# yangzhaojason/DualDiff

Hardware: AMD Instinct MI355X
Metric: denoising-steps/sec, 6-view 224×400 fp16, 50-step DDIM @ 1/2/4/8 MI355X (higher is better)
Workload: dtype fp16; 1 GPU; BASELINE configs[1]: 6-view 224x400 (28x50 latents) multiview UNet + 2 ControlNet branches (ORS panorama + ORS-3D, SFA on), CFG 2.0 -> 12 view-instances/scene, DDIM-50 schedule, random-init weights; scenes_per_gpu=1, parallelism=scene-sharded x1 (no data-path collective), hip_graph=True, streams=3, invariant_conditioning=recomputed every step

## Files before the change

### dualdiff_amd/_native.py

```python
import ctypes
import os

import torch
from ctypes import (POINTER, Structure, c_char_p, c_float, c_int32, c_int64, c_uint32, c_void_p)

from . import _build

DD_F16, DD_BF16, DD_F32 = 0, 1, 2
DD_EPI_NONE, DD_EPI_GEGLU, DD_EPI_SILU = 0, 1, 2


class GemmDesc(Structure):
    _fields_ = [
        ("a", c_void_p), ("a2", c_void_p), ("lda", c_int64), ("lda2", c_int64), ("k1", c_int32),
        ("rows", c_int32), ("n", c_int32), ("k", c_int32),
        ("w", c_void_p), ("bias", c_void_p), ("rowvec", c_void_p),
        ("rows_per_inst", c_int32), ("ld_rowvec", c_int32),
        ("res", c_void_p), ("ldres", c_int64),
        ("out", c_void_p), ("ldc", c_int64),
        ("alpha", c_float), ("accumulate", c_int32), ("epilogue", c_int32),
        ("conv", c_int32), ("hin", c_int32), ("win", c_int32), ("cin", c_int32),
        ("hv", c_int32), ("wv", c_int32), ("hout", c_int32), ("wout", c_int32), ("stride", c_int32),
        ("dtype", c_int32), ("tile", c_int32), ("split_k", c_int32),
        ("ws", c_void_p), ("ws_bytes", c_int64),
# ... 69 lines not shown
    "dd_gemm_num_tiles": (c_int32, []),
    "dd_gemm_tile_id": (c_int32, [c_int32]),
    "dd_gemm_kernel_name": (c_char_p, [POINTER(GemmDesc)]),
    "dd_gemm_conv_pad": (c_int32, [POINTER(GemmDesc), c_int32, c_void_p]),
    "dd_gemm_conv_pad_workspace_bytes": (c_int64, [POINTER(GemmDesc), c_int32]),
    "dd_gemm_conv_pad_kernel_name": (c_char_p, [POINTER(GemmDesc), c_int32]),
    "dd_groupnorm_nhwc": (c_int32, [c_void_p, c_int32, c_void_p, c_int32, c_void_p, c_void_p, c_void_p,
                                    c_int32, c_int32, c_int32, c_float, c_int32, c_int32,
                                    c_void_p, c_int64, c_void_p]),
    "dd_groupnorm_workspace_bytes": (c_int64, [c_int32, c_int32]),
    "dd_groupnorm_is_fused": (c_int32, [c_int32, c_int32, c_int32]),
    "dd_layernorm": (c_int32, [c_void_p, c_void_p, c_void_p, c_void_p, c_int64, c_int32, c_float,
                               c_int32, c_void_p]),
    "dd_attention": (c_int32, [POINTER(AttnDesc), c_void_p]),
    "dd_attention_kernel_name": (c_char_p, [POINTER(AttnDesc)]),
    "dd_add": (c_int32, [c_void_p, c_void_p, c_void_p, c_void_p, c_int64, c_int32, c_void_p]),
    "dd_scale": (c_int32, [c_void_p, c_void_p, c_float, c_int64, c_int32, c_void_p]),
    "dd_probe_spin": (c_int32, [c_void_p, c_uint32, c_void_p]),
    "dd_groupnorm_splitk": (c_int32, [c_void_p, c_int32, c_void_p, c_void_p, c_int32, c_void_p, c_int64, c_void_p,
                                      c_void_p, c_void_p, c_void_p, c_int32, c_int32, c_int32, c_int32, c_float, c_int32,
                                      c_int32, c_void_p]),
    "dd_xattn320": (c_int32, [POINTER(XAttnDesc), c_void_p]),
    "dd_nchw_to_nhwc_views": (c_int32, [c_void_p, c_void_p, c_int32, c_int32, c_int32, c_int32, c_int32, c_int32, c_int32,
                                        c_void_p]),
    "dd_fourier_embed_strided": (c_int32, [c_void_p, c_void_p, c_int64, c_int32, POINTER(c_float), c_int32, c_int32,
                                           c_int32, c_int32, c_int32, c_int64, c_int64, c_int64, c_int64, c_void_p]),
    "dd_box_tokens": (c_int32, [POINTER(BoxTokensDesc), c_void_p]),
    "dd_ctx_assemble": (c_int32, [c_void_p, c_void_p, c_void_p, c_void_p, c_void_p, c_int32, c_int32, c_int32, c_int32,
                                  c_int32, c_int32, c_int32, c_int32, c_void_p]),
    "dd_gemm8": (c_int32, [POINTER(Gemm8Desc), c_void_p]),
    "dd_rowquant_fp8": (c_int32, [c_void_p, c_void_p, c_void_p, c_void_p, c_void_p, c_int64, c_int32, c_int64, c_float,
                                  c_int32, c_void_p]),
    "dd_xattn_pack_weight": (c_int32, [c_void_p, c_void_p, c_int32, c_void_p]),
    "dd_silu": (c_int32, [c_void_p, c_void_p, c_int64, c_int32, c_void_p]),
    "dd_nchw_to_nhwc": (c_int32, [c_void_p, c_void_p, c_int32, c_int32, c_int32, c_int32, c_int32, c_void_p]),
    "dd_nhwc_to_nchw": (c_int32, [c_void_p, c_void_p, c_int32, c_int32, c_int32, c_int32, c_int32, c_void_p]),
    "dd_timestep_embedding": (c_int32, [c_void_p, c_void_p, c_int32, c_int32, c_int32, c_float,
                                        c_int32, c_void_p]),
    "dd_cfg_unipc_step": (c_int32, [c_void_p, c_void_p, c_void_p, c_void_p, c_void_p, c_void_p, c_void_p, c_void_p,
                                    c_float, c_int64, c_int32, c_void_p]),
    "dd_softmax_rows": (c_int32, [c_void_p, c_void_p, c_int64, c_int32, c_int64, c_int64, c_int32, c_void_p]),
    "dd_ors_project": (c_int32, [c_void_p, c_void_p, c_void_p, c_void_p, c_void_p, c_int32, c_int32, c_int32,
                                 c_float, c_int32, c_int32, c_int32, c_void_p]),
    "dd_fourier_embed": (c_int32, [c_void_p, c_void_p, c_int64, c_int32, POINTER(c_float), c_int32, c_int32,
                                   c_int32, c_int32, c_void_p]),
    "dd_conv3x3_small_cout": (c_int32, [c_void_p, c_void_p, c_void_p, c_void_p, c_int32, c_int32,
                                        c_int32, c_int32, c_int32, c_int32, c_void_p]),
    "dd_vae_posterior": (c_int32, [c_void_p, c_void_p, c_void_p, c_void_p, c_void_p, c_int32, c_int32, c_int32, c_float,
                                   c_int32, c_int32, c_void_p]),
    "dd_image_quantize_u8": (c_int32, [c_void_p, c_void_p, c_int32, c_int32, c_int32, c_int32, c_int32, c_void_p]),
    "dd_image_resample_u8": (c_int32, [c_void_p, c_void_p, c_int32, c_int32, c_int32, c_int32, c_int32, c_void_p, c_void_p,
                                       c_int32, c_void_p, c_void_p, c_int32, c_int32, c_int32, c_int32, c_int32, c_int32,
                                       c_int32, c_int32, c_void_p]),
    "dd_image_load_u8": (c_int32, [c_void_p, c_void_p, c_int32, c_int32, c_int32, c_int32, c_int32, c_void_p, c_void_p,
                                   c_int32, c_void_p, c_void_p, c_int32, c_void_p, c_int32, c_int32, c_void_p]),
    "dd_clip_embed": (c_int32, [c_void_p, c_void_p, c_void_p, c_void_p, c_void_p, c_int32, c_int32, c_int32, c_int32,
                                c_int32, c_int32, c_void_p]),
    "dd_causal_attention": (c_int32, [c_void_p, c_void_p, c_void_p, c_void_p, c_int64, c_int64, c_int64, c_int64,
                                      c_int64, c_int64, c_int64, c_int64, c_int32, c_int32, c_int32, c_int32, c_float,
                                      c_int32, c_void_p]),
    "dd_conv3x3_thin": (c_int32, [c_void_p, c_void_p, c_void_p, c_void_p, c_int32, c_int32, c_int32, c_int32, c_int32,
                                  c_int32, c_int32, c_int32, c_void_p]),
    "dd_cfg_ddim_step": (c_int32, [c_void_p, c_void_p, c_void_p, c_void_p, c_void_p, c_float,
                                   c_int64, c_int32, c_void_p]),
    "dd_cfg_ddim_step_given": (c_int32, [c_void_p, c_void_p, c_void_p, c_void_p, c_void_p, c_float, c_void_p, c_void_p,
                                         c_void_p, c_void_p, c_int32, c_int64, c_int64, c_int32, c_void_p]),
# ... 55 lines not shown
```

### dualdiff_amd/csrc/xattn.hip

```cpp
#include "dd_common.h"
#include <type_traits>

namespace {

constexpr int XC = 320;
constexpr int XH = 8;
constexpr int XD = 40;
constexpr int XR = 80;
constexpr int XW = 10;
constexpr int XPITCH = XC + 8;
constexpr int XLK = 128;
constexpr size_t kActBytes = 53 * 1024;

struct XAttnParams {
  const void* x; int64_t ldx;
  const void* res; int64_t ldres;
  const void* wq; const void* wo;
  const void* bo;
  const void* k; const void* v;
  int64_t ldk, ldv;
  int64_t k_is, k_hs, v_is, v_hs;
  void* out; int64_t ldo;
  void* ln_out; int64_t ld_ln; const void* ln_g; const void* ln_b; float ln_eps;
  int inst, n, lk;
// ... 343 lines not shown
#pragma unroll
  for (int tm = 0; tm < 5; ++tm) {
    float a = 0.f;
#pragma unroll
    for (int w = 0; w < XW; ++w) a += red2[(tm * 16 + c) * XW + w];
    const float rstd = 1.0f / sqrtf(a * (1.0f / XC) + p.ln_eps);
    const int row = tm * 16 + c;
    if (row >= nrows) continue;
#pragma unroll
    for (int tn = 0; tn < 2; ++tn) {
      const int ch = wave * 32 + tn * 16 + g * 4;
      V4 o4;
#pragma unroll
      for (int r = 0; r < 4; ++r)
        o4[r] = (T)(((float)yv[tn][tm][r] - mean[tm]) * rstd * (float)lng[tn][r] + (float)lnb4[tn][r]);
      *reinterpret_cast<V4*>(lnb + (int64_t)row * p.ld_ln + ch) = o4;
    }
  }
}

constexpr size_t kXSmem = kActBytes + (size_t)4 * XC * 32 * 2;

template <typename T>
int launch_xattn(const XAttnParams& p, hipStream_t s) {
  static_assert(2 * (2 * XLK * XD * 2) == 4 * XC * 32, "two K/V buffers = the four weight slots");
  static_assert(XR * 41 * 16 <= 52 * 1024 && 53 * 1024 == (int)kActBytes && XPITCH * 2 == 41 * 16, "activation tile");
  auto kern = dd_xattn320_kernel<T>;
  static std::atomic<uint64_t> attr_done{0};
  dd_ensure_dyn_lds(reinterpret_cast<const void*>(kern), kXSmem, attr_done);
  hipLaunchKernelGGL(kern, dim3(p.inst * p.tiles), dim3(64 * XW), kXSmem, s, p);
  return dd_check_launch();
}

}

namespace {
template <typename T>
__global__ void dd_xattn_pack_kernel(const T* __restrict__ w, T* __restrict__ out) {
  const int q = blockIdx.x * blockDim.x + threadIdx.x;
  if (q >= 10 * XC * 4) return;
  const int ks = q / (XC * 4), rem = q - ks * (XC * 4);
  const int n = rem >> 2, pos = rem & 3;
  const int src = ks * 32 + ((pos ^ ((n >> 2) & 3)) << 3);
  dd_st16(out + (int64_t)q * 8, dd_ld16(w + (int64_t)n * XC + src));
}
}

extern "C" int dd_xattn_pack_weight(const void* w, void* packed, int32_t dtype, dd_stream_t stream) {
  if (!w || !packed || !dd_aligned16(w) || !dd_aligned16(packed)) return DD_ERR_BAD_ARG;
  if (dtype != DD_F16 && dtype != DD_BF16) return DD_ERR_BAD_ARG;
  dd_clear_error();
  const int chunks = 10 * XC * 4;
  return dd_dispatch16(dtype, [&](auto t) {
    using T = typename decltype(t)::type;
    hipLaunchKernelGGL(dd_xattn_pack_kernel<T>, dim3((chunks + 255) / 256), dim3(256), 0, dd_stream(stream),
                       (const T*)w, (T*)packed);
    return dd_check_launch();
  });
}

extern "C" int dd_xattn320(const dd_xattn_desc* d, dd_stream_t stream) {
  if (!d || !d->x || !d->wq || !d->wo || !d->bo || !d->k || !d->v || !d->out) return DD_ERR_BAD_ARG;
  if (d->instances <= 0 || d->rows_per_inst <= 0 || d->lk <= 0) return DD_ERR_BAD_ARG;
  if (d->channels != XC || d->heads != XH) return DD_ERR_UNSUPPORTED;
  if (d->lk > XLK) return DD_ERR_UNSUPPORTED;
  if (d->dtype != DD_F16 && d->dtype != DD_BF16) return DD_ERR_BAD_ARG;
// ... 26 lines not shown
```

### dualdiff_amd/networks/layers.py

```python
import math

import torch
import torch.nn as nn

from .. import ops as O


CACHE_EPOCH = [0]


class _Cached(nn.Module):

    def _drop_cache(self):
        CACHE_EPOCH[0] += 1
        for k in [k for k in self.__dict__ if k.startswith("_pk_")]:
            del self.__dict__[k]

    def _apply(self, fn, *a, **k):
        self._drop_cache()
        return super()._apply(fn, *a, **k)

    def _load_from_state_dict(self, *a, **k):
        self._drop_cache()
        return super()._load_from_state_dict(*a, **k)
# ... 66 lines not shown
    if not p.is_contiguous():
        if not x.is_cuda or x.dtype not in (torch.float16, torch.bfloat16):
            p = p.contiguous()
        else:
            return O.nchw_to_nhwc(x), m, h, w
    return p.reshape(m * h * w, c), m, h, w


def as_nchw_view(x2d, m, h, w):
    return x2d.view(m, h, w, x2d.shape[1]).permute(0, 3, 1, 2)


class Linear(_Cached):

    def __init__(self, in_features, out_features, bias=True, conv=False):
        super().__init__()
        self.in_features, self.out_features, self.conv = in_features, out_features, conv
        shape = (out_features, in_features, 1, 1) if conv else (out_features, in_features)
        self.weight = nn.Parameter(torch.empty(shape))
        self.bias = nn.Parameter(torch.empty(out_features)) if bias else None

    @property
    def w2d(self):
        if "_pk_w" not in self.__dict__:
            self.__dict__["_pk_w"] = _pad_cols(self.weight.detach().reshape(self.out_features, -1))
        return self.__dict__["_pk_w"]

    @property
    def wx(self):
        ver = (self.weight.data_ptr(), self.weight._version)
        hit = self.__dict__.get("_pk_wx")
        if hit is None or (hit[1] != ver and not torch.cuda.is_current_stream_capturing()):
            hit = self.__dict__["_pk_wx"] = (O.xattn_pack_weight(self.w2d), ver)
        return hit[0]

    fp8_mfma = False

    @property
    def w8p(self):
        if "_pk_w8p" not in self.__dict__:
            self.__dict__["_pk_w8p"] = O.quantize_fp8_padded(self.w2d)
        return self.__dict__["_pk_w8p"]

    def run(self, x2d, ln_next=None, **kw):
        if ln_next is not None and ln_producer_ok(self, ln_next, kw):
            w = self.w2d
            out = O.gemm(x2d, w, self.bias, ln_out=(ln_next.weight, ln_next.bias, ln_next.eps), **kw)
            out._ln_cache = (ln_next, out._ln_out)
            return out
        w = self.w2d
        if w.shape[1] != self.in_features:
            x2d = torch.nn.functional.pad(x2d, (0, w.shape[1] - x2d.shape[1]))
        return O.gemm(x2d, w, self.bias, **kw)

    def run_ln(self, x2d, norm, **kw):
        if self.fp8_mfma and fp8_mfma_ok(norm, self.in_features, self.out_features, x2d) \
                and set(kw) <= {"epilogue"} and kw.get("epilogue", O.DD_EPI_NONE) in (O.DD_EPI_NONE, O.DD_EPI_GEGLU):
            a8, sa = O.rowquant_fp8(x2d, (norm.weight, norm.bias, norm.eps))
            w8, sw = self.w8p
            return O.gemm8(a8, sa, w8, sw, self.bias, dtype=x2d.dtype, geglu=kw.get("epilogue") == O.DD_EPI_GEGLU)
        if not ln_fold_ok(norm, self.in_features, self.out_features, x2d):
            return self.run(norm.run(x2d), **kw)
        w, ln = fold_layernorm(self.__dict__, "_pk_ln", norm, [self.weight], [self.bias])
        return O.gemm(x2d, w, None, ln=ln, **kw)

    def forward(self, x):
# ... 86 lines not shown
def ln_fold_ok(norm, k, n=None, x=None):
    if LN_FOLD == "0" or not isinstance(norm, LayerNorm) or k not in (320, 640, 1280):
        return False
    if LN_FOLD == "stats":
        return x is not None and getattr(x, "_ln_stats", None) is not None
    return LN_FOLD == "all" or (n is not None and n <= k)


def want_ln_stats():
    return LN_FOLD == "stats"


LN_PRODUCER = __import__("os").environ.get("DD_LN_PRODUCER", "1") != "0"


def ln_producer_ok(lin, norm, kw):
    if not LN_PRODUCER or not isinstance(norm, LayerNorm) or lin.out_features != 320:
        return False
    if LN_FOLD != "0":
        return False
    if lin.w2d.shape[1] % 64 or kw.get("a2") is not None and kw["a2"].shape[1] % 64:
        return False
    bad = ("ln", "ln_stats", "head_major", "out_f32", "accumulate", "rowvec", "out", "tile", "split_k")
    return not any(kw.get(k) for k in bad) and kw.get("epilogue", O.DD_EPI_NONE) == O.DD_EPI_NONE \
        and kw.get("alpha", 1.0) == 1.0


def fp8_mfma_ok(norm, k, n, x2d):
    return isinstance(norm, LayerNorm) and k in (640, 1280) and n >= 3 * k and x2d.is_contiguous() \
        and getattr(x2d, "_ln_cache", None) is None


XATTN_FUSED = __import__("os").environ.get("DD_XATTN_FUSED", "1") != "0"


HEAD_MAJOR = __import__("os").environ.get("DD_ATTN_HEAD_MAJOR", "1") != "0"


def fold_layernorm(cache, key, norm, weights, biases):
    params = [norm.weight, norm.bias] + list(weights) + [b for b in biases if b is not None]
    ver = tuple((t._version, t.data_ptr()) for t in params)
    hit = cache.get(key)
    if hit is not None and hit[0] == ver:
        return hit[1], hit[2]
    with torch.no_grad():
        w = torch.cat([t.detach().reshape(t.shape[0], -1) for t in weights], dim=0).float()
        b = torch.cat([(bb.detach().float() if bb is not None else torch.zeros(t.shape[0], device=t.device))
                       for t, bb in zip(weights, biases)])
        wp = (w * norm.weight.detach().float()[None, :]).to(weights[0].dtype).contiguous()
        colsum = wp.float().sum(dim=1).contiguous()
        lnb = (w @ norm.bias.detach().float() + b).contiguous()
    cache[key] = (ver, wp, (colsum, lnb, norm.eps))
    return wp, (colsum, lnb, norm.eps)


class _Dropout(nn.Module):

    def forward(self, x):
        return x


class Timesteps(nn.Module):
    def __init__(self, num_channels, flip_sin_to_cos, downscale_freq_shift):
        super().__init__()
        self.num_channels, self.flip_sin_to_cos = num_channels, flip_sin_to_cos
        self.downscale_freq_shift = downscale_freq_shift
# ... 160 lines not shown
    def run_self(self, x2d, batch, lq, res=None, norm=None, ln_stats=False, ln_next=None):
        c, hd = self.inner_dim, self.heads
        if HEAD_MAJOR and self.to_q.bias is None:
            qkv = self.project_qkv(x2d, norm, head_major=True)
            o = O.attention(qkv[:hd], qkv[hd:2 * hd], qkv[2 * hd:], batch, lq, lq, hd, self.dim_head,
                            q_prescaled=True)
        else:
            qkv = self.project_qkv(x2d, norm)
            o = O.attention(qkv[:, :c], qkv[:, c:2 * c], qkv[:, 2 * c:], batch, lq, lq, hd,
                            self.dim_head, self.scale)
        return self.to_out[0].run(o, res=res, ln_stats=ln_stats, ln_next=ln_next)

    def run_cross(self, x2d, batch, lq, ctx2d, lk, res=None, kv=None, norm=None, ln_stats=False, ln_next=None):
        c = self.inner_dim
        pre = self.__dict__.pop("_kv_prefetched", None)
        if kv is None and pre is not None and pre[0] is ctx2d:
            kv, side = pre[1], pre[2]
            if side is not None:
                torch.cuda.current_stream().wait_stream(side)
                if not torch.cuda.is_current_stream_capturing():
                    kv.record_stream(torch.cuda.current_stream())
        if kv is None:
            kv = self.project_kv(ctx2d)
        lk_dev = lk_dev_for(ctx2d, lk)
        if XATTN_FUSED and O.xattn320_ok(c, self.heads, lk, x2d.shape[0]) and self.to_q.in_features == c and self.to_q.bias is None \
                and not ln_stats and LN_FOLD == "0":
            xn = x2d if norm is None else norm.run(x2d)
            lno = (ln_next.weight, ln_next.bias, ln_next.eps) if LN_PRODUCER and isinstance(ln_next, LayerNorm) else None
            out = O.xattn320(xn, self.to_q.wx, self.to_out[0].wx, self.to_out[0].bias, kv[:, :c], kv[:, c:], batch, lq,
                             lk, self.scale, res=res, ln_out=lno, lk_dev=lk_dev)
            if lno is not None:
                out._ln_cache = (ln_next, out._ln_out)
            return out
        q_hm = HEAD_MAJOR and self.to_q.bias is None
        kw = {"head_major": self._hm(self.heads)} if q_hm else {}
        q = self.to_q.run(x2d, **kw) if norm is None else self.to_q.run_ln(x2d, norm, **kw)
        o = O.attention(q, kv[:, :c], kv[:, c:], batch, lq, lk, self.heads, self.dim_head, self.scale,
                        q_prescaled=q_hm, lk_dev=lk_dev)
        return self.to_out[0].run(o, res=res, ln_stats=ln_stats, ln_next=ln_next)

    def forward(self, hidden_states, encoder_hidden_states=None, attention_mask=None, **kw):
        return self.processor(self, hidden_states, encoder_hidden_states=encoder_hidden_states,
                              attention_mask=attention_mask, **kw)


def enable_fp8_weights(model, on=True, mfma=True):
    if not mfma:
        raise NotImplementedError("the weights-only fp8 form (row-panel GEMM family) was removed in round 5; use mfma=True")
    n = 0
    for mod in model.modules():
        if isinstance(mod, Attention):
            mod.fp8_mfma = bool(on)
            mod._drop_cache()
            n += 1
        elif isinstance(mod, GEGLU):
            mod.proj.fp8_mfma = bool(on)
            mod.proj._drop_cache()
    return n


def prefetch_cross_kv(model, ctx2d, side):
    main = torch.cuda.current_stream()
    side.wait_stream(main)
    with torch.cuda.stream(side):
        for blk in model.modules():
            mod = getattr(blk, "attn2", None) if isinstance(blk, BasicTransformerBlock) else None
# ... 309 lines not shown
```

### dualdiff_amd/ops.py

```python
import collections as _collections
import ctypes
import os as _os

import torch

from . import _native, _timer, _workspace, tuning
from ._native import DD_BF16, DD_EPI_GEGLU, DD_EPI_NONE, DD_EPI_SILU, DD_F16, AttnDesc, Gemm8Desc, GemmDesc, XAttnDesc
from ._timer import KernelTimer, _stream, set_timer
from ._workspace import workspace, workspace_owner
from .tuning import (CHALLENGE_TILES, TUNE_TABLE_PATH, forget_tuned, load_tuned, save_tuned,
                     tune_candidates, tuned_table)

_THIN_CONV = _os.environ.get("DD_THIN_CONV", "1") != "0"
GN_SPLITK = _os.environ.get("DD_GN_SPLITK", "0") == "1"
LN_OUT_TILE = int(_os.environ.get("DD_LN_OUT_TILE", "0"))
XATTN_MAX_WGS = int(_os.environ.get("DD_XATTN_MAX_WGS", "256"))
CAUSAL_ATTN_MAX_L = 128
_ZERO_BIAS = {}
_FDT = {torch.float16: 0, torch.bfloat16: 1, torch.float32: 2}


def _dtype_code(dtype):
    if dtype == torch.float16:
        return DD_F16
    if dtype == torch.bfloat16:
        return DD_BF16
    raise TypeError("dualdiff_amd ops take fp16 / bf16 tensors, got %s" % dtype)


def _dt(t):
    return _dtype_code(t.dtype)


def _tname(code):
    return "f16" if code == DD_F16 else "bf16"


def _need_gpu(*ts):
    for t in ts:
        if t is not None and not t.is_cuda:
            raise RuntimeError("dualdiff_amd ops run on the GPU only (got a %s tensor); "
                               "there is no CPU fallback" % t.device)


def _ptr(t):
    return ctypes.c_void_p(t.data_ptr()) if t is not None else None


def _forget_derived(t):
# ... 541 lines not shown
    d.x, d.ldx = x.data_ptr(), x.stride(0)
    if res is not None:
        res = _rows2d(res)
        d.res, d.ldres = res.data_ptr(), res.stride(0)
    d.wq, d.wo = wqp.data_ptr(), wop.data_ptr()
    if bo is None:
        key = (x.dtype, x.device)
        if key not in _ZERO_BIAS:
            _ZERO_BIAS[key] = torch.zeros(320, dtype=x.dtype, device=x.device)
        bo = _ZERO_BIAS[key]
    d.bo = bo.data_ptr()
    d.k, d.ldk, d.k_inst_stride, d.k_head_stride = kv_operand(k)
    d.v, d.ldv, d.v_inst_stride, d.v_head_stride = kv_operand(v)
    d.out, d.ldo = out.data_ptr(), out.stride(0)
    d.instances, d.rows_per_inst, d.lk = int(instances), int(rows_per_inst), int(lk)
    d.channels, d.heads, d.scale, d.dtype = 320, 8, float(scale), _dt(x)
    d.lk_dev = lk_dev.data_ptr() if lk_dev is not None else None
    second = None
    if ln_out is not None:
        g_, b_, eps_ = ln_out
        _need_gpu(g_, b_)
        second = torch.empty((rows, 320), dtype=x.dtype, device=x.device)
        d.ln_out, d.ld_ln_out = second.data_ptr(), 320
        d.ln_gamma, d.ln_beta, d.ln_eps = g_.data_ptr(), b_.data_ptr(), float(eps_)
    _timer.launch("xattn320", lib.dd_xattn320, ctypes.byref(d), _stream(),
                  book=lambda: ("dd_xattn320_kernel", 4.0 * rows * 320 * 320 + 4.0 * rows * lk * 320,
                                2.0 * (rows * 320 * (2 + (1 if res is not None else 0) + (1 if second is not None else 0))
                                       + 2 * 320 * 320 + 2 * instances * lk * 320)))
    if second is not None:
        out._ln_out = second
    return out


def add(a, b, c=None, out=None):
    lib = _native.load()
    _need_gpu(a, b, c, out)
    out = _out_or_new(out, a, a.dtype, a.device, "add")
    _timer.launch("add", lib.dd_add, _ptr(a), _ptr(b), _ptr(c), _ptr(out), a.numel(), _dt(a), _stream(),
                  book=lambda: ("dd_add", 0.0, 2.0 * a.numel() * (3 + (1 if c is not None else 0))))
    return out


def scale(x, s, out=None):
    lib = _native.load()
    _need_gpu(x, out)
    out = _out_or_new(out, x, x.dtype, x.device, "scale")
    _native.check(lib.dd_scale(_ptr(x), _ptr(out), s, x.numel(), _dt(x), _stream()), "scale")
    return out


def silu(x, out=None):
    lib = _native.load()
    _need_gpu(x, out)
    out = _out_or_new(out, x, x.dtype, x.device, "silu")
    _native.check(lib.dd_silu(_ptr(x), _ptr(out), x.numel(), _dt(x), _stream()), "silu")
    return out


def nchw_to_nhwc(x, c_pad=None, views=1):
    lib = _native.load()
    _need_gpu(x)
    m, c, h, wt = x.shape
    if wt % views:
        raise ValueError("nchw_to_nhwc: width %d is not %d views" % (wt, views))
    c_pad = c if c_pad is None else c_pad
    x = x.contiguous()
# ... 339 lines not shown
```

### include/dualdiff_hip.h

```cpp
#ifndef DUALDIFF_HIP_H
#define DUALDIFF_HIP_H

#include <stdint.h>

#ifdef __cplusplus
extern "C" {
#endif

#define DD_ABI_VERSION 4

enum { DD_F16 = 0, DD_BF16 = 1 };

enum {
  DD_OK = 0,
  DD_ERR_BAD_ARG = -1,
  DD_ERR_UNSUPPORTED = -2,
  DD_ERR_LAUNCH = -3,
  DD_ERR_WORKSPACE = -4
};

typedef void* dd_stream_t;

int dd_abi_version(void);
int64_t dd_desc_size(int which);
// ... 77 lines not shown
  float scale;
  const int32_t* kv_batch_map;
  int32_t accumulate;
  int32_t dtype;
  int32_t variant;
  int64_t q_head_stride, k_head_stride, v_head_stride;
  int32_t q_prescaled;
  const int32_t* kv_batch_map2;
  const int32_t* lk_dev;
} dd_attn_desc;

int dd_attention(const dd_attn_desc* d, dd_stream_t stream);
const char* dd_attention_kernel_name(const dd_attn_desc* d);

typedef struct dd_xattn_desc {
  const void* x; int64_t ldx;
  const void* res; int64_t ldres;
  const void* wq; const void* wo; const void* bo;
  const void* k; const void* v; int64_t ldk, ldv;
  int64_t k_inst_stride, k_head_stride, v_inst_stride, v_head_stride;
  void* out; int64_t ldo;
  int32_t instances, rows_per_inst, lk;
  int32_t channels, heads;
  float scale;
  int32_t dtype;
  void* ln_out; int64_t ld_ln_out;
  const void* ln_gamma; const void* ln_beta; float ln_eps;
  const int32_t* lk_dev;
} dd_xattn_desc;

int dd_xattn320(const dd_xattn_desc* d, dd_stream_t stream);
int dd_xattn_pack_weight(const void* w, void* packed, int32_t dtype, dd_stream_t stream);

int dd_add(const void* a, const void* b, const void* c, void* y, int64_t n,
           int32_t dtype, dd_stream_t stream);
int dd_scale(const void* x, void* y, float s, int64_t n, int32_t dtype, dd_stream_t stream);
int dd_silu(const void* x, void* y, int64_t n, int32_t dtype, dd_stream_t stream);

int dd_nchw_to_nhwc(const void* x, void* y, int32_t m, int32_t c, int32_t hw,
                    int32_t c_pad, int32_t dtype, dd_stream_t stream);
int dd_nhwc_to_nchw(const void* x, void* y, int32_t m, int32_t c, int32_t hw,
                    int32_t ldx, int32_t dtype, dd_stream_t stream);

int dd_timestep_embedding(const float* t, void* out, int32_t n, int32_t dim,
                          int32_t flip_sin_to_cos, float freq_shift,
                          int32_t dtype, dd_stream_t stream);

#define DD_F32 2
int dd_fourier_embed(const void* x, void* out, int64_t rows, int32_t dims, const float* freqs,
                     int32_t num_freqs, int32_t include_input, int32_t in_dtype, int32_t out_dtype,
                     dd_stream_t stream);

int dd_nchw_to_nhwc_views(const void* x, void* y, int32_t m, int32_t c, int32_t h, int32_t w, int32_t views,
                          int32_t c_pad, int32_t dtype, dd_stream_t stream);
int dd_fourier_embed_strided(const void* x, void* out, int64_t rows, int32_t dims, const float* freqs,
                             int32_t num_freqs, int32_t include_input, int32_t in_dtype, int32_t out_dtype,
                             int32_t inner, int64_t stride_outer, int64_t stride_inner, int64_t stride_dim,
                             int64_t out_ld, dd_stream_t stream);
typedef struct dd_box_tokens_desc {
  const void* points; const int64_t* classes; const uint8_t* masks;
  const void* class_tokens; const void* null_pos; const void* null_class;
  void* pos; void* cat; void* cls_out;
  int32_t rows, points_per_box, num_freqs, include_input, class_token_dim, cls_offset;
  int64_t ld_cat;
  int32_t normalize, points_dtype, dtype;
  int32_t n_classes;
// ... 91 lines not shown
```

Before: 94.34 steps/s.

## Fuse LayerNorm, Q projection and cross-attention into one kernel for 1280-channel levels

Adds a HIP kernel that loads a row tile, applies LayerNorm in LDS, computes the per-head Q projection with MFMA while streaming pre-packed weights through a ring buffer, then runs softmax attention against short K/V in the same workgroup. It is enabled by default for 1280-channel cross-attention when the workgroup count is small. This removes the separate LN+Q GEMM launch, the Q round-trip through global memory, and the separate attention launch at the low-resolution UNet levels. In exchange each workgroup recomputes LayerNorm for its rows once per head (8x redundant LN and X reads), and small grids may underfill the GPU.

Result: no change. 94.45 steps/s, median of 2 (+0.1%).

```diff
diff --git a/dualdiff_amd/_native.py b/dualdiff_amd/_native.py
--- a/dualdiff_amd/_native.py
+++ b/dualdiff_amd/_native.py
@@ -125,6 +125,9 @@
     "dd_rowquant_fp8": (c_int32, [c_void_p, c_void_p, c_void_p, c_void_p, c_void_p, c_int64, c_int32, c_int64, c_float,
                                   c_int32, c_void_p]),
     "dd_xattn_pack_weight": (c_int32, [c_void_p, c_void_p, c_int32, c_void_p]),
+    "dd_xattn_q": (c_int32, [POINTER(XAttnDesc), c_void_p]),
+    "dd_xattn_q_tile_rows": (c_int32, [c_int32, c_int32]),
+    "dd_xattn_q_pack_weight": (c_int32, [POINTER(XAttnDesc), c_void_p]),
     "dd_silu": (c_int32, [c_void_p, c_void_p, c_int64, c_int32, c_void_p]),
     "dd_nchw_to_nhwc": (c_int32, [c_void_p, c_void_p, c_int32, c_int32, c_int32, c_int32, c_int32, c_void_p]),
     "dd_nhwc_to_nchw": (c_int32, [c_void_p, c_void_p, c_int32, c_int32, c_int32, c_int32, c_int32, c_void_p]),
diff --git a/dualdiff_amd/csrc/xattn.hip b/dualdiff_amd/csrc/xattn.hip
--- a/dualdiff_amd/csrc/xattn.hip
+++ b/dualdiff_amd/csrc/xattn.hip
@@ -399,6 +399,379 @@
   return dd_check_launch();
 }
 
+
+struct XQParams {
+  const void* x; int64_t ldx;
+  const void* wq;
+  const void* ln_g; const void* ln_b; float ln_eps;
+  const void* k; const void* v;
+  int64_t ldk, ldv, k_is, k_hs, v_is, v_hs;
+  void* out; int64_t ldo;
+  void* q_out; int64_t ldq;
+  int inst, n, lk, tiles;
+  const int32_t* lk_dev;
+  float qscale;
+};
+
+__device__ __forceinline__ void xwait_vmcnt_n(int n) {
+  switch (n) {
+    case 0: xwait_vmcnt<0>(); break;
+    case 1: xwait_vmcnt<1>(); break;
+    case 2: xwait_vmcnt<2>(); break;
+    case 3: xwait_vmcnt<3>(); break;
+    case 4: xwait_vmcnt<4>(); break;
+    case 5: xwait_vmcnt<5>(); break;
+    case 6: xwait_vmcnt<6>(); break;
+    default: xwait_vmcnt<7>(); break;
+  }
+}
+
+template <int C, int MB, int NS>
+struct XQGeom {
+  static constexpr int D = C / 8, NW = D / 16, R = MB * 16, NST = C / 32, CH = C / 8;
+  static constexpr int LPR = C / 40, RPW = 64 / LPR;
+  static constexpr int XBYTES = R * C * 2;
+  static constexpr int XI = XBYTES / 1024 / NW;
+  static constexpr int QP = D + 8;
+  static constexpr int KCH = D / 8 + 1;
+  static constexpr int KI = XLK * KCH * 16 / 1024;
+  static constexpr int QBYTES = R * QP * 2, KBYTES = XLK * QP * 2;
+  static constexpr int SMEM = XBYTES + NW * NS * 1024;
+  static_assert(XBYTES % (1024 * NW) == 0 && (XLK * KCH * 16) % 1024 == 0, "whole DMA instructions");
+  static_assert(QBYTES + 2 * KBYTES <= SMEM && SMEM <= 160 * 1024, "LDS budget");
+  static_assert(NS >= 3 && NS <= 9 && R % RPW == 0 && MB <= NW, "geometry");
+};
+
+template <typename T, int C, int MB, int NS>
+__global__ __launch_bounds__(64 * (C / 128))
+void dd_xattn_q_kernel(const XQParams p) {
+  using G = XQGeom<C, MB, NS>;
+  using V8 = typename dd_vec<T>::v8;
+  using V4 = typename dd_vec<T>::v4;
+  constexpr int D = G::D, NW = G::NW, R = G::R, NST = G::NST, CH = G::CH, QP = G::QP;
+  extern __shared__ __attribute__((aligned(16))) unsigned char smem[];
+  T* xs = reinterpret_cast<T*>(smem);
+  unsigned char* ringb = smem + G::XBYTES;
+
+  const int tid = threadIdx.x;
+  const int lane = tid & 63;
+  const int wave = __builtin_amdgcn_readfirstlane(tid >> 6);
+  const int c = lane & 15;
+  const int g = lane >> 4;
+  const int lk = p.lk_dev ? min(max(__builtin_amdgcn_readfirstlane(*p.lk_dev), 1), p.lk) : p.lk;
+
+  const int head = blockIdx.x & (XH - 1);
+  const int it = blockIdx.x >> 3;
+  const int inst = it / p.tiles;
+  const int t = it - inst * p.tiles;
+  const int r0 = t * R;
+  const int nrows = min(R, p.n - r0);
+  const int64_t grow0 = (int64_t)inst * p.n + r0;
+
+  const __amdgpu_buffer_rsrc_t rs_x = __builtin_amdgcn_make_buffer_rsrc(
+      const_cast<T*>(reinterpret_cast<const T*>(p.x) + grow0 * p.ldx), 0,
+      (uint32_t)(((int64_t)(nrows - 1) * p.ldx + C) * sizeof(T)), 0x00020000);
+  const __amdgpu_buffer_rsrc_t rs_w = __builtin_amdgcn_make_buffer_rsrc(
+      const_cast<T*>(reinterpret_cast<const T*>(p.wq) + (int64_t)head * D * C), 0, D * C * sizeof(T), 0x00020000);
+  const __amdgpu_buffer_rsrc_t rs_k = __builtin_amdgcn_make_buffer_rsrc(
+      const_cast<T*>(reinterpret_cast<const T*>(p.k) + (int64_t)inst * p.k_is + (int64_t)head * p.k_hs), 0,
+      (uint32_t)(((int64_t)(lk - 1) * p.ldk + D) * sizeof(T)), 0x00020000);
+  const __amdgpu_buffer_rsrc_t rs_v = __builtin_amdgcn_make_buffer_rsrc(
+      const_cast<T*>(reinterpret_cast<const T*>(p.v) + (int64_t)inst * p.v_is + (int64_t)head * p.v_hs), 0,
+      (uint32_t)(((int64_t)(lk - 1) * p.ldv + D) * sizeof(T)), 0x00020000);
+
+#pragma unroll
+  for (int i = 0; i < G::XI; ++i) {
+    const int wi = i * NW + wave;
+    const int q = wi * 64 + lane;
+    const int row = q / CH, pos = q - row * CH;
+    const uint32_t voff = row < nrows ? (uint32_t)(row * (int)p.ldx * 2 + ((pos ^ (row & 7)) << 4)) : X_OOB;
+    xdma16(rs_x, voff, 0, smem + wi * 1024);
+  }
+  unsigned char* myring = ringb + wave * (NS * 1024);
+  const uint32_t wvoff = (uint32_t)(wave * 1024 + lane * 16);
+  auto issue_w = [&](int s) { xdma16(rs_w, wvoff, (uint32_t)(s * (NW * 1024)), myring + (s % NS) * 1024); };
+#pragma unroll
+  for (int s = 0; s < NS - 1; ++s) issue_w(s);
+  const int sub = lane % G::LPR;
+  u32x4 gam[5], bet[5];
+#pragma unroll
+  for (int i = 0; i < 5; ++i) {
+    gam[i] = dd_ld16(reinterpret_cast<const T*>(p.ln_g) + (sub + i * G::LPR) * 8);
+    bet[i] = dd_ld16(reinterpret_cast<const T*>(p.ln_b) + (sub + i * G::LPR) * 8);
+  }
+  auto lds_barrier = [&]() {
+    asm volatile("s_waitcnt lgkmcnt(0)" ::: "memory");
+    __builtin_amdgcn_s_barrier();
+    asm volatile("" ::: "memory");
+  };
+  xwait_vmcnt<0>();
+  lds_barrier();
+#pragma unroll 1
+  for (int pp = wave; pp < R / G::RPW; pp += NW) {
+    const int row = pp * G::RPW + lane / G::LPR;
+    T* xr = xs + row * C;
+    float f[5][8];
+    float s = 0.f;
+#pragma unroll
+    for (int i = 0; i < 5; ++i) {
+      dd_unpack8<T>(dd_ld16(xr + (((sub + i * G::LPR) ^ (row & 7)) << 3)), f[i]);
+#pragma unroll
+      for (int e = 0; e < 8; ++e) s += f[i][e];
+    }
+#pragma unroll
+    for (int o = G::LPR / 2; o > 0; o >>= 1) s += __shfl_xor(s, o, 64);
+    const float mean = s * (1.0f / (float)C);
+    float ss = 0.f;
+#pragma unroll
+    for (int i = 0; i < 5; ++i)
+#pragma unroll
+      for (int e = 0; e < 8; ++e) { const float d = f[i][e] - mean; ss += d * d; }
+#pragma unroll
+    for (int o = G::LPR / 2; o > 0; o >>= 1) ss += __shfl_xor(ss, o, 64);
+    const float rstd = rsqrtf(ss * (1.0f / (float)C) + p.ln_eps);
+#pragma unroll
+    for (int i = 0; i < 5; ++i) {
+      float ga[8], be[8], o[8];
+      dd_unpack8<T>(gam[i], ga);
+      dd_unpack8<T>(bet[i], be);
+#pragma unroll
+      for (int e = 0; e < 8; ++e) o[e] = (f[i][e] - mean) * rstd * ga[e] + be[e];
+      dd_st16(xr + (((sub + i * G::LPR) ^ (row & 7)) << 3), dd_pack8<T>(o));
+    }
+  }
+  lds_barrier();
+
+  f32x4 acc[MB];
+#pragma unroll
+  for (int mb = 0; mb < MB; ++mb) acc[mb] = f32x4{0.f, 0.f, 0.f, 0.f};
+#pragma unroll
+  for (int s = 0; s < NST; ++s) {
+    if (s > 0) {
+      const int left = NST - 1 - s;
+      xwait_vmcnt_n(left < NS - 2 ? left : NS - 2);
+    }
+    if (s + NS - 1 < NST) issue_w(s + NS - 1);
+    const T* slot = reinterpret_cast<const T*>(myring + (s % NS) * 1024);
+    const V8 wf = dd_as_v8<T>(dd_ld16(slot + c * 32 + ((g ^ ((c >> 1) & 3)) << 3)));
+    V8 xf[MB];
+#pragma unroll
+    for (int mb = 0; mb < MB; ++mb)
+      xf[mb] = dd_as_v8<T>(dd_ld16(xs + (mb * 16 + c) * C + (((s * 4 + g) ^ (c & 7)) << 3)));
+#pragma unroll
+    for (int mb = 0; mb < MB; ++mb) acc[mb] = dd_mfma16(wf, xf[mb], acc[mb]);
+  }
+  lds_barrier();
+
+  T* Qs = reinterpret_cast<T*>(smem);
+  T* Ks = reinterpret_cast<T*>(smem + G::QBYTES);
+  T* Vs = reinterpret_cast<T*>(smem + G::QBYTES + G::KBYTES);
+  const int kpad = ((lk + 31) >> 5) << 5;
+#pragma unroll
+  for (int i = 0; i < (G::KI + NW - 1) / NW; ++i) {
+    const int wi = i * NW + wave;
+    if (wi < G::KI && (wi * 64) / G::KCH < kpad) {
+      const int q = wi * 64 + lane;
+      const int key = q / G::KCH, ch = q - key * G::KCH;
+      const bool in = key < lk && ch < D / 8;
+      xdma16(rs_k, in ? (uint32_t)((key * (int)p.ldk + ch * 8) * 2) : X_OOB, 0, reinterpret_cast<unsigned char*>(Ks) + wi * 1024);
+      xdma16(rs_v, in ? (uint32_t)((key * (int)p.ldv + ch * 8) * 2) : X_OOB, 0, reinterpret_cast<unsigned char*>(Vs) + wi * 1024);
+    }
+  }
+#pragma unroll
+  for (int mb = 0; mb < MB; ++mb) {
+    V4 q4;
+#pragma unroll
+    for (int r = 0; r < 4; ++r) q4[r] = (T)(acc[mb][r] * p.qscale);
+    *reinterpret_cast<V4*>(Qs + (mb * 16 + c) * QP + wave * 16 + g * 4) = q4;
+    if (p.q_out && mb * 16 + c < nrows)
+      *reinterpret_cast<V4*>(reinterpret_cast<T*>(p.q_out) + (grow0 + mb * 16 + c) * p.ldq + head * D + wave * 16 + g * 4) = q4;
+  }
+  xwait_vmcnt<0>();
+  lds_barrier();
+  if (wave >= MB) return;
+  const int rb = wave;
+  if (rb * 16 >= nrows) return;
+  const int nkb = (lk + 15) >> 4;
+  constexpr int QS = (D + 31) / 32;
+  const u32x4 zero4 = {0u, 0u, 0u, 0u};
+  V8 qf[QS];
+#pragma unroll
+  for (int st = 0; st < QS; ++st)
+    qf[st] = dd_as_v8<T>(st * 4 + g < D / 8 ? dd_ld16(Qs + (rb * 16 + c) * QP + (st * 4 + g) * 8) : zero4);
+  f32x4 s[8];
+#pragma unroll
+  for (int b = 0; b < 8; ++b) {
+    s[b] = f32x4{0.f, 0.f, 0.f, 0.f};
+    if (b < nkb) {
+      const T* krow = Ks + (b * 16 + c) * QP;
+#pragma unroll
+      for (int st = 0; st < QS; ++st) {
+        const V8 kf = dd_as_v8<T>(st * 4 + g < D / 8 ? dd_ld16(krow + (st * 4 + g) * 8) : zero4);
+        s[b] = dd_mfma16(kf, qf[st], s[b]);
+      }
+    }
+  }
+  float mx = -INFINITY;
+#pragma unroll
+  for (int b = 0; b < 8; ++b) {
+    if (b < nkb) {
+#pragma unroll
+      for (int r = 0; r < 4; ++r) {
+        if (b * 16 + g * 4 + r >= lk) s[b][r] = -INFINITY;
+        mx = fmaxf(mx, s[b][r]);
+      }
+    }
+  }
+  mx = fmaxf(mx, __shfl_xor(mx, 16, 64));
+  mx = fmaxf(mx, __shfl_xor(mx, 32, 64));
+  float sum = 0.f;
+  V8 pf[4];
+#pragma unroll
+  for (int j = 0; j < 4; ++j) {
+    V8 pv;
+#pragma unroll
+    for (int hb = 0; hb < 2; ++hb) {
+      if (j * 2 + hb < nkb) {
+#pragma unroll
+        for (int r = 0; r < 4; ++r) {
+          const float pe = __builtin_amdgcn_exp2f(s[j * 2 + hb][r] - mx);
+          const T pt = (T)pe;
+          sum += (float)pt;
+          pv[hb * 4 + r] = pt;
+        }
+      } else {
+#pragma unroll
+        for (int r = 0; r < 4; ++r) pv[hb * 4 + r] = (T)0.f;
+      }
+    }
+    pf[j] = pv;
+  }
+  sum += __shfl_xor(sum, 16, 64);
+  sum += __shfl_xor(sum, 32, 64);
+  const float inv = 1.0f / sum;
+  const uint32_t vaddr = (uint32_t)(uintptr_t)(__attribute__((address_space(3))) const void*)(Vs + (g * 4 + (c >> 2)) * QP + (c & 3) * 4);
+  T* outb = reinterpret_cast<T*>(p.out) + (grow0 + rb * 16 + c) * p.ldo + head * D;
+#pragma unroll
+  for (int dt = 0; dt < D / 16; ++dt) {
+    f32x4 o = f32x4{0.f, 0.f, 0.f, 0.f};
+    u32x2 f[8];
+    asm volatile(
+        "ds_read_b64_tr_b16 %0, %8 offset:%9\n\t"
+        "ds_read_b64_tr_b16 %1, %8 offset:%10\n\t"
+        "ds_read_b64_tr_b16 %2, %8 offset:%11\n\t"
+        "ds_read_b64_tr_b16 %3, %8 offset:%12\n\t"
+        "ds_read_b64_tr_b16 %4, %8 offset:%13\n\t"
+        "ds_read_b64_tr_b16 %5, %8 offset:%14\n\t"
+        "ds_read_b64_tr_b16 %6, %8 offset:%15\n\t"
+        "ds_read_b64_tr_b16 %7, %8 offset:%16\n\t"
+        "s_waitcnt lgkmcnt(0)"
+        : "=&v"(f[0]), "=&v"(f[1]), "=&v"(f[2]), "=&v"(f[3]), "=&v"(f[4]), "=&v"(f[5]), "=&v"(f[6]), "=&v"(f[7])
+        : "v"(vaddr + (uint32_t)(dt * 32)),
+          "n"((0 * 32) * QP * 2), "n"((0 * 32 + 16) * QP * 2), "n"((1 * 32) * QP * 2), "n"((1 * 32 + 16) * QP * 2),
+          "n"((2 * 32) * QP * 2), "n"((2 * 32 + 16) * QP * 2), "n"((3 * 32) * QP * 2), "n"((3 * 32 + 16) * QP * 2)
+        : "memory");
+#pragma unroll
+    for (int j = 0; j < 4; ++j) {
+      if (j * 2 < nkb) {
+        V8 vf;
+        __builtin_memcpy(&vf, &f[2 * j], 8);
+        __builtin_memcpy(reinterpret_cast<char*>(&vf) + 8, &f[2 * j + 1], 8);
+        o = dd_mfma16(vf, pf[j], o);
+      }
+    }
+    if (rb * 16 + c < nrows) {
+      V4 o4;
+#pragma unroll
+      for (int r = 0; r < 4; ++r) o4[r] = (T)(o[r] * inv);
+      *reinterpret_cast<V4*>(outb + dt * 16 + g * 4) = o4;
+    }
+  }
+}
+
+template <typename T, int C, int MB, int NS>
+int launch_xattn_q(XQParams p, hipStream_t s) {
+  using G = XQGeom<C, MB, NS>;
+  auto kern = dd_xattn_q_kernel<T, C, MB, NS>;
+  static std::atomic<uint64_t> attr_done{0};
+  dd_ensure_dyn_lds(reinterpret_cast<const void*>(kern), G::SMEM, attr_done);
+  p.tiles = (p.n + G::R - 1) / G::R;
+  if ((int64_t)p.inst * p.tiles * XH > 0x7fffffffLL) return DD_ERR_UNSUPPORTED;
+  hipLaunchKernelGGL(kern, dim3(p.inst * p.tiles * XH), dim3(64 * G::NW), G::SMEM, s, p);
+  return dd_check_launch();
+}
+
+template <typename T>
+__global__ void dd_xattn_q_pack_kernel(const T* __restrict__ w, T* __restrict__ out, int C) {
+  const int q = blockIdx.x * blockDim.x + threadIdx.x;
+  if (q >= C * (C / 8)) return;
+  const int D = C / 8, NW = D / 16, NST = C / 32;
+  const int pos = q & 3, row = (q >> 2) & 15;
+  int rest = q >> 6;
+  const int nb = rest % NW; rest /= NW;
+  const int s = rest % NST;
+  const int head = rest / NST;
+  const int n = head * D + nb * 16 + row;
+  dd_st16(out + (int64_t)q * 8, dd_ld16(w + (int64_t)n * C + s * 32 + ((pos ^ ((row >> 1) & 3)) << 3)));
+}
+
+}
+
+extern "C" int dd_xattn_q_tile_rows(int32_t channels, int32_t rows_per_inst) {
+  if (channels == 640) return 32;
+  if (channels == 1280) return rows_per_inst <= 32 ? 32 : 48;
+  return 0;
+}
+
+extern "C" int dd_xattn_q_pack_weight(const dd_xattn_desc* d, dd_stream_t stream) {
+  if (!d || !d->wq || !d->out || !dd_aligned16(d->wq) || !dd_aligned16(d->out)) return DD_ERR_BAD_ARG;
+  if (d->dtype != DD_F16 && d->dtype != DD_BF16) return DD_ERR_BAD_ARG;
+  if (d->channels != 640 && d->channels != 1280) return DD_ERR_UNSUPPORTED;
+  dd_clear_error();
+  const int channels = d->channels;
+  const int chunks = channels * (channels / 8);
+  return dd_dispatch16(d->dtype, [&](auto t) {
+    using T = typename decltype(t)::type;
+    hipLaunchKernelGGL(dd_xattn_q_pack_kernel<T>, dim3((chunks + 255) / 256), dim3(256), 0, dd_stream(stream),
+                       (const T*)d->wq, (T*)d->out, channels);
+    return dd_check_launch();
+  });
+}
+
+extern "C" int dd_xattn_q(const dd_xattn_desc* d, dd_stream_t stream) {
+  if (!d || !d->x || !d->wq || !d->k || !d->v || !d->out || !d->ln_gamma || !d->ln_beta) return DD_ERR_BAD_ARG;
+  if (d->res || d->wo || d->bo) return DD_ERR_BAD_ARG;
+  if (d->instances <= 0 || d->rows_per_inst <= 0 || d->lk <= 0) return DD_ERR_BAD_ARG;
+  if ((d->channels != 640 && d->channels != 1280) || d->heads != XH) return DD_ERR_UNSUPPORTED;
+  if (d->lk > XLK) return DD_ERR_UNSUPPORTED;
+  if (d->dtype != DD_F16 && d->dtype != DD_BF16) return DD_ERR_BAD_ARG;
+  if ((d->ldx & 7) || (d->ldk & 7) || (d->ldv & 7) || (d->ldo & 3)) return DD_ERR_BAD_ARG;
+  if (d->ldx < d->channels || d->ldo < d->channels) return DD_ERR_BAD_ARG;
+  if (!dd_aligned16(d->x) || !dd_aligned16(d->wq) || !dd_aligned16(d->k) || !dd_aligned16(d->v) || !dd_aligned16(d->out) ||
+      !dd_aligned16(d->ln_gamma) || !dd_aligned16(d->ln_beta)) return DD_ERR_BAD_ARG;
+  if (d->ln_out && (!dd_aligned16(d->ln_out) || (d->ld_ln_out & 3) || d->ld_ln_out < d->channels)) return DD_ERR_BAD_ARG;
+  if (d->lk_dev && (reinterpret_cast<uintptr_t>(d->lk_dev) & 3u)) return DD_ERR_BAD_ARG;
+  const int dh = d->channels / XH;
+  XQParams p{};
+  p.x = d->x; p.ldx = d->ldx; p.wq = d->wq;
+  p.ln_g = d->ln_gamma; p.ln_b = d->ln_beta; p.ln_eps = d->ln_eps;
+  p.k = d->k; p.v = d->v; p.ldk = d->ldk; p.ldv = d->ldv;
+  p.k_is = d->k_inst_stride; p.k_hs = d->k_head_stride; p.v_is = d->v_inst_stride; p.v_hs = d->v_head_stride;
+  if ((p.k_is & 7) || (p.k_hs & 7) || (p.v_is & 7) || (p.v_hs & 7)) return DD_ERR_BAD_ARG;
+  if (((int64_t)(d->lk - 1) * d->ldk + dh) * 2 >= (1ll << 31) || ((int64_t)(d->lk - 1) * d->ldv + dh) * 2 >= (1ll << 31) ||
+      (int64_t)48 * d->ldx * 2 >= (1ll << 31)) return DD_ERR_UNSUPPORTED;
+  p.out = d->out; p.ldo = d->ldo;
+  p.q_out = d->ln_out; p.ldq = d->ld_ln_out;
+  p.inst = d->instances; p.n = d->rows_per_inst; p.lk = d->lk; p.lk_dev = d->lk_dev;
+  p.qscale = d->scale * 1.44269504088896340736f;
+  const int tr = dd_xattn_q_tile_rows(d->channels, d->rows_per_inst);
+  dd_clear_error();
+  return dd_dispatch16(d->dtype, [&](auto t) {
+    using T = typename decltype(t)::type;
+    if (d->channels == 640) return launch_xattn_q<T, 640, 2, 7>(p, dd_stream(stream));
+    if (tr == 32) return launch_xattn_q<T, 1280, 2, 7>(p, dd_stream(stream));
+    return launch_xattn_q<T, 1280, 3, 4>(p, dd_stream(stream));
+  });
 }
 
 namespace {
diff --git a/dualdiff_amd/networks/layers.py b/dualdiff_amd/networks/layers.py
--- a/dualdiff_amd/networks/layers.py
+++ b/dualdiff_amd/networks/layers.py
@@ -122,6 +122,14 @@
         hit = self.__dict__.get("_pk_wx")
         if hit is None or (hit[1] != ver and not torch.cuda.is_current_stream_capturing()):
             hit = self.__dict__["_pk_wx"] = (O.xattn_pack_weight(self.w2d), ver)
+        return hit[0]
+
+    @property
+    def wxq(self):
+        ver = (self.weight.data_ptr(), self.weight._version)
+        hit = self.__dict__.get("_pk_wxq")
+        if hit is None or (hit[1] != ver and not torch.cuda.is_current_stream_capturing()):
+            hit = self.__dict__["_pk_wxq"] = (O.xattn_q_pack_weight(self.w2d), ver)
         return hit[0]
 
     fp8_mfma = False
@@ -274,6 +282,15 @@
 
 
 XATTN_FUSED = __import__("os").environ.get("DD_XATTN_FUSED", "1") != "0"
+XATTN_Q = __import__("os").environ.get("DD_XATTN_Q", "1") != "0"
+XATTN_Q_LEVELS = (1280,)
+
+
+def xattn_q_ok(attn, batch, lq, lk, norm, ln_stats):
+    c = attn.inner_dim
+    return XATTN_Q and c in XATTN_Q_LEVELS and LN_FOLD == "0" and not ln_stats and isinstance(norm, LayerNorm) \
+        and attn.to_q.bias is None and attn.to_q.in_features == c and not attn.fp8_mfma and not attn.to_q.fp8_mfma \
+        and O.xattn_q_ok(c, attn.heads, lk, batch, lq)
 
 
 HEAD_MAJOR = __import__("os").environ.get("DD_ATTN_HEAD_MAJOR", "1") != "0"
@@ -500,6 +517,11 @@
             if lno is not None:
                 out._ln_cache = (ln_next, out._ln_out)
             return out
+        if xattn_q_ok(self, batch, lq, lk, norm, ln_stats) and getattr(x2d, "_ln_cache", None) is None \
+                and x2d.shape[1] == c and x2d.dtype == self.to_q.weight.dtype and kv.dtype == x2d.dtype:
+            o = O.xattn_q(x2d, (norm.weight, norm.bias, norm.eps), self.to_q.wxq, kv[:, :c], kv[:, c:], batch, lq, lk,
+                          self.scale, lk_dev=lk_dev)
+            return self.to_out[0].run(o, res=res, ln_stats=ln_stats, ln_next=ln_next)
         q_hm = HEAD_MAJOR and self.to_q.bias is None
         kw = {"head_major": self._hm(self.heads)} if q_hm else {}
         q = self.to_q.run(x2d, **kw) if norm is None else self.to_q.run_ln(x2d, norm, **kw)
diff --git a/dualdiff_amd/ops.py b/dualdiff_amd/ops.py
--- a/dualdiff_amd/ops.py
+++ b/dualdiff_amd/ops.py
@@ -15,6 +15,7 @@
 GN_SPLITK = _os.environ.get("DD_GN_SPLITK", "0") == "1"
 LN_OUT_TILE = int(_os.environ.get("DD_LN_OUT_TILE", "0"))
 XATTN_MAX_WGS = int(_os.environ.get("DD_XATTN_MAX_WGS", "256"))
+XATTN_Q_MAX_WGS = int(_os.environ.get("DD_XATTN_Q_MAX_WGS", "256"))
 CAUSAL_ATTN_MAX_L = 128
 _ZERO_BIAS = {}
 _FDT = {torch.float16: 0, torch.bfloat16: 1, torch.float32: 2}
@@ -622,6 +623,85 @@
     return out
 
 
+def xattn_q_tile_rows(c, rows_per_inst):
+    if int(c) == 640:
+        return 32
+    if int(c) == 1280:
+        return 32 if int(rows_per_inst) <= 32 else 48
+    return 0
+
+
+def xattn_q_wgs(c, instances, rows_per_inst):
+    tr = xattn_q_tile_rows(c, rows_per_inst)
+    return int(instances) * ((int(rows_per_inst) + tr - 1) // tr) * 8 if tr else 0
+
+
+def xattn_q_ok(c, heads, lk, instances=None, rows_per_inst=None):
+    if int(c) not in (640, 1280) or int(heads) != 8 or not 0 < int(lk) <= 128:
+        return False
+    if instances is not None and xattn_q_wgs(c, instances, rows_per_inst) > XATTN_Q_MAX_WGS:
+        return False
+    return True
+
+
+def xattn_q_pack_weight(w):
+    if w.dim() != 2 or w.shape[0] != w.shape[1] or w.shape[0] not in (640, 1280) or not w.is_contiguous():
+        raise ValueError("xattn_q weights must be contiguous (640, 640) or (1280, 1280)")
+    _need_gpu(w)
+    lib = _native.load()
+    packed = torch.empty(w.numel(), dtype=w.dtype, device=w.device)
+    d = XAttnDesc()
+    d.wq, d.out, d.channels, d.dtype = w.data_ptr(), packed.data_ptr(), int(w.shape[0]), _dt(w)
+    _native.check(lib.dd_xattn_q_pack_weight(ctypes.byref(d), _stream()), "xattn_q_pack_weight")
+    return packed
+
+
+def xattn_q(x, ln, wq, k, v, instances, rows_per_inst, lk, scale, *, out=None, lk_dev=None, q_out=None):
+    lib = _native.load()
+    g_, b_, eps_ = ln
+    _need_gpu(x, wq, k, v, out, lk_dev, g_, b_, q_out)
+    _check_lk_dev(lk_dev)
+    x = _rows2d(x)
+    rows = instances * rows_per_inst
+    c = x.shape[1]
+    if x.shape[0] != rows or c not in (640, 1280):
+        raise ValueError("xattn_q: x must be (instances * rows_per_inst, 640 | 1280)")
+    if g_.numel() != c or b_.numel() != c or g_.dtype != x.dtype or b_.dtype != x.dtype \
+            or not g_.is_contiguous() or not b_.is_contiguous():
+        raise ValueError("xattn_q: LayerNorm weight / bias must be contiguous (C,) of x's dtype")
+    wqp = wq if wq.dim() == 1 and wq.numel() == c * c else xattn_q_pack_weight(wq)
+    if wqp.dtype != x.dtype:
+        raise TypeError("xattn_q: weight dtype differs from x")
+    d = XAttnDesc()
+    d.x, d.ldx = x.data_ptr(), x.stride(0)
+    d.wq = wqp.data_ptr()
+    for name, t in (("k", k), ("v", v)):
+        t = _rows2d(t)
+        if t.shape[0] != instances * lk or t.shape[1] < c or t.dtype != x.dtype:
+            raise ValueError("xattn_q: K / V must be (instances * lk, >= C) of x's dtype")
+        setattr(d, name, t.data_ptr())
+        setattr(d, "ld" + name, t.stride(0))
+        setattr(d, name + "_inst_stride", lk * t.stride(0))
+        setattr(d, name + "_head_stride", c // 8)
+    out = _rows2d(_out_or_new(out, (rows, c), x.dtype, x.device, "xattn_q"))
+    if out.shape != (rows, c):
+        raise ValueError("xattn_q: out must be (rows, C)")
+    d.out, d.ldo = out.data_ptr(), out.stride(0)
+    d.instances, d.rows_per_inst, d.lk = int(instances), int(rows_per_inst), int(lk)
+    d.channels, d.heads, d.scale, d.dtype = c, 8, float(scale), _dt(x)
+    d.ln_gamma, d.ln_beta, d.ln_eps = g_.data_ptr(), b_.data_ptr(), float(eps_)
+    d.lk_dev = lk_dev.data_ptr() if lk_dev is not None else None
+    if q_out is not None:
+        q_out = _rows2d(q_out)
+        if q_out.shape != (rows, c) or q_out.dtype != x.dtype:
+            raise ValueError("xattn_q: q_out must be (rows, C) of x's dtype")
+        d.ln_out, d.ld_ln_out = q_out.data_ptr(), q_out.stride(0)
+    _timer.launch("xattn_q", lib.dd_xattn_q, ctypes.byref(d), _stream(),
+                  book=lambda: ("dd_xattn_q_kernel", 2.0 * rows * c * c + 4.0 * rows * lk * c,
+                                2.0 * (2 * rows * c + c * c + 2 * instances * lk * c)))
+    return out
+
+
 def add(a, b, c=None, out=None):
     lib = _native.load()
     _need_gpu(a, b, c, out)
diff --git a/include/dualdiff_hip.h b/include/dualdiff_hip.h
--- a/include/dualdiff_hip.h
+++ b/include/dualdiff_hip.h
@@ -133,6 +133,10 @@
 int dd_xattn320(const dd_xattn_desc* d, dd_stream_t stream);
 int dd_xattn_pack_weight(const void* w, void* packed, int32_t dtype, dd_stream_t stream);
 
+int dd_xattn_q(const dd_xattn_desc* d, dd_stream_t stream);
+int dd_xattn_q_tile_rows(int32_t channels, int32_t rows_per_inst);
+int dd_xattn_q_pack_weight(const dd_xattn_desc* d, dd_stream_t stream);
+
 int dd_add(const void* a, const void* b, const void* c, void* y, int64_t n,
            int32_t dtype, dd_stream_t stream);
 int dd_scale(const void* x, void* y, float s, int64_t n, int32_t dtype, dd_stream_t stream);
```
